# StevenWang30/R-PCC

Hardware: AMD Instinct MI355X
Metric: frames/s (64E, 64x2048 range img), projection->segmentation->model->quantise (higher is better)
Workload: dtype f32

## Files before the change

include/rpcc_hip.h:

```cpp
#ifndef RPCC_HIP_H
#define RPCC_HIP_H

#include <stddef.h>
#include <stdint.h>

#ifdef __cplusplus
extern "C" {
#endif

#define RPCC_OK 0
#define RPCC_ERR_ARG (-1)
#define RPCC_ERR_HIP (-2)
#define RPCC_MAX_CLUSTERS 254
#define RPCC_MAX_BATCH 65535
#define RPCC_INFO_INTS 8
#define RPCC_FPS_BRUTEFORCE 1
#define RPCC_FPS_FMA1 2
#define RPCC_FPS_FMA2 4
#define RPCC_FPS_TIE_CUDA 8



#define RPCC_ABI_VERSION 105
int rpcc_version(void);
// ... 18 lines not shown
int rpcc_beam_index_build(const double *angles, int H, void *out);
size_t rpcc_project_beams_scratch_bytes(int64_t total, int B, int P);
int rpcc_project_beams(const float *points, int point_stride_bytes, const int64_t *offsets, int64_t total, int B, rpcc_geom g,
                       const void *beams_dev, float *ri, void *scratch, size_t scratch_bytes, void *stream);
int rpcc_project_beams_check(const float *xyz, int64_t total, rpcc_geom g, const void *beams_dev, uint64_t *counts, void *stream);

size_t rpcc_intensity_scratch_bytes(int B, int P);
int rpcc_intensity_encode(const float *rows, const int64_t *offsets, int64_t total, int B, rpcc_geom g, const float *ri, float scale,
                          uint8_t *payload, int64_t payload_stride, int32_t *nbytes, uint8_t *image, float *owner_intensity, int32_t *orphans,
                          void *scratch, size_t scratch_bytes, void *stream);
int rpcc_intensity_decode(const uint8_t *payload, int64_t payload_stride, const int32_t *nbytes, const void *labels, int label_bytes, int B,
                          int P, float *intensity, int32_t *status, void *stream);

#define RPCC_STREAM_E_SUBPIXEL 11
size_t rpcc_subpixel_scratch_bytes(int B, int P);
int rpcc_subpixel_encode(const float *rows, const int64_t *offsets, int64_t total, int B, rpcc_geom g, const float *ri, int bits,
                         uint8_t *payload, int64_t payload_stride, int32_t *nbytes, uint8_t *codes, int32_t *orphans, void *scratch,
                         size_t scratch_bytes, void *stream);
int rpcc_subpixel_decode(const uint8_t *payload, int64_t payload_stride, const int32_t *nbytes, const void *labels, int label_bytes,
                         const float *ri_rec, const double *tables, int H, int W, int B, float *points, int32_t *status, void *stream);

int rpcc_ground_ransac(const float *ri, const float *tm, int B, int P, uint32_t seed, const int64_t *frame_ids,
                       double *ground, int32_t *inliers, void *stream);

int rpcc_ground_mask(const float *ri, const float *tm, const double *ground, double threshold, int B, int H, int W,
                     float *temp, int32_t *info, void *fps_table, void *stream);
size_t rpcc_fps_table_bytes(int B, int H, int W);

int rpcc_fps_xyz(int B, int N, int M, const float *points, float *temp, int32_t *idx, void *stream);

int rpcc_fps_range(const float *ri, const float *tm, float *temp, const int32_t *info, int B, int H, int W, int M,
                   int32_t *cen_pix, float *centers, int flags,
                   const void *fps_table , void *stream);

int rpcc_fps_xyz_bruteforce(int B, int N, int M, const float *points, float *temp, int32_t *idx, void *stream);
int rpcc_fps_xyz_mode(int B, int N, int M, const float *points, float *temp, int32_t *idx, int flags, void *stream);
int rpcc_fps_xyz_probe(int B, int N, const float *points, int32_t *marks, void *stream);

int rpcc_assign(const float *ri, const float *tm, const double *ground, const float *centers, int B, int H, int W,
                int M, uint8_t *seg, void *stream);

int rpcc_point_model(const float *ri, const uint8_t *seg, const double *ground, int B, int P, int M, float *model,
                     int32_t *counts, void *ws, void *stream);

size_t rpcc_plane_workspace_bytes(int B, int P, int M);
int rpcc_plane_model(const float *ri, const float *tm, const uint8_t *seg, const double *ground, int B, int P, int M,
// ... 164 lines not shown
```

r-pcc_amd/_lib.py:

```python
import ctypes as C
import os

import torch

_HERE = os.path.dirname(os.path.abspath(__file__))
LIB_PATH = os.environ.get("RPCC_HIP_LIB") or os.path.join(_HERE, "lib", "librpcc_hip.so")


MAX_GROUPS = 4


class Geom(C.Structure):
    _fields_ = [("H", C.c_int32), ("W", C.c_int32), ("horizontal_fov", C.c_float), ("vertical_max", C.c_float),
                ("vertical_min", C.c_float)]


class BatchIO(C.Structure):
    _fields_ = [("xyz", C.c_void_p), ("offsets", C.c_void_p), ("total", C.c_int64), ("tm", C.c_void_p),
                ("ground", C.c_void_p), ("ground_seed", C.c_int64), ("frame_ids", C.c_void_p), ("ri", C.c_void_p),
                ("seg", C.c_void_p), ("cen_pix", C.c_void_p), ("centers", C.c_void_p), ("model", C.c_void_p),
                ("counts", C.c_void_p), ("q16", C.c_void_p), ("nnz", C.c_void_p), ("info", C.c_void_p),
                ("flags", C.c_int32), ("timer", C.c_void_p), ("model_method", C.c_int32), ("plane_cos_cut", C.c_double),
                ("plane_seed", C.c_int64), ("nonuniform", C.c_void_p), ("salience", C.c_void_p), ("key_point_map", C.c_void_p),
                ("point_stride_bytes", C.c_int32)]
# ... 40 lines not shown
    pass


_VP, _I, _I64, _F, _D = C.c_void_p, C.c_int, C.c_int64, C.c_float, C.c_double
_SIGS = {
    "rpcc_version": (C.c_int, []),
    "rpcc_last_error": (C.c_char_p, []),
    "rpcc_project_scratch_bytes": (C.c_size_t, [_I64, _I, _I]),
    "rpcc_project_fastpath_check": (C.c_int, [_VP, _I64, Geom, _VP, _VP]),
    "rpcc_project": (C.c_int, [_VP, _VP, _I64, _I, Geom, _VP, _VP, C.c_size_t, _VP]),
    "rpcc_project_strided": (C.c_int, [_VP, _I, _VP, _I64, _I, Geom, _VP, _VP, C.c_size_t, _VP]),
    "rpcc_beam_index_bytes": (C.c_size_t, [_I]),
    "rpcc_beam_index_build": (C.c_int, [_VP, _I, _VP]),
    "rpcc_project_beams_scratch_bytes": (C.c_size_t, [_I64, _I, _I]),
    "rpcc_project_beams": (C.c_int, [_VP, _I, _VP, _I64, _I, Geom, _VP, _VP, _VP, C.c_size_t, _VP]),
    "rpcc_project_beams_check": (C.c_int, [_VP, _I64, Geom, _VP, _VP, _VP]),
    "rpcc_intensity_scratch_bytes": (C.c_size_t, [_I, _I]),
    "rpcc_intensity_encode": (C.c_int, [_VP, _VP, _I64, _I, Geom, _VP, _F, _VP, _I64, _VP, _VP, _VP, _VP, _VP, C.c_size_t, _VP]),
    "rpcc_intensity_decode": (C.c_int, [_VP, _I64, _VP, _VP, _I, _I, _I, _VP, _VP, _VP]),
    "rpcc_subpixel_scratch_bytes": (C.c_size_t, [_I, _I]),
    "rpcc_subpixel_encode": (C.c_int, [_VP, _VP, _I64, _I, Geom, _VP, _I, _VP, _I64, _VP, _VP, _VP, _VP, C.c_size_t, _VP]),
    "rpcc_subpixel_decode": (C.c_int, [_VP, _I64, _VP, _VP, _I, _VP, _VP, _I, _I, _I, _VP, _VP, _VP]),
    "rpcc_ground_ransac": (C.c_int, [_VP, _VP, _I, _I, C.c_uint32, _VP, _VP, _VP, _VP]),
    "rpcc_ground_mask": (C.c_int, [_VP, _VP, _VP, _D, _I, _I, _I, _VP, _VP, _VP, _VP]),
    "rpcc_fps_table_bytes": (C.c_size_t, [_I, _I, _I]),
    "rpcc_fps_xyz": (C.c_int, [_I, _I, _I, _VP, _VP, _VP, _VP]),
    "rpcc_fps_xyz_bruteforce": (C.c_int, [_I, _I, _I, _VP, _VP, _VP, _VP]),
    "rpcc_fps_xyz_mode": (C.c_int, [_I, _I, _I, _VP, _VP, _VP, _I, _VP]),
    "rpcc_fps_xyz_probe": (C.c_int, [_I, _I, _VP, _VP, _VP]),
    "rpcc_fps_range": (C.c_int, [_VP, _VP, _VP, _VP, _I, _I, _I, _I, _VP, _VP, _I, _VP, _VP]),
    "rpcc_assign": (C.c_int, [_VP, _VP, _VP, _VP, _I, _I, _I, _I, _VP, _VP]),
    "rpcc_point_model": (C.c_int, [_VP, _VP, _VP, _I, _I, _I, _VP, _VP, _VP, _VP]),
    "rpcc_predict_quantize": (C.c_int, [_VP, _VP, _VP, _VP, _VP, _VP, _F, _I, _I, _I, _VP, _VP, _VP, _VP, _VP, _VP]),
    "rpcc_intra_predict": (C.c_int, [_VP, _VP, _VP, _I, _I, _I, _VP, _VP]),
    "rpcc_assign_wide": (C.c_int, [_VP, _VP, _VP, _VP, _I, _I, _I, _I, _VP, _VP]),
    "rpcc_point_model_wide": (C.c_int, [_VP, _VP, _VP, _I, _I, _I, _VP, _VP, _VP, _VP]),
    "rpcc_predict_quantize_wide": (C.c_int, [_VP, _VP, _VP, _VP, _VP, _VP, _F, _I, _I, _I, _VP, _VP, _VP, _VP, _VP, _VP]),
    "rpcc_intra_predict_wide": (C.c_int, [_VP, _VP, _VP, _I, _I, _I, _VP, _VP]),
    "rpcc_extract_features_wide": (C.c_int, [_VP, _VP, _I, _I, _I, _I, _I, _I, _I, _I, _VP, _VP, _VP]),
    "rpcc_salience_wide": (C.c_int, [_VP, _VP, C.POINTER(C.c_int32), C.POINTER(C.c_float), _I, _I, _I, _I, _I, _VP, _VP, _VP]),
    "rpcc_plane_model_wide": (C.c_int, [_VP, _VP, _VP, _VP, _I, _I, _I, _D, C.c_uint32, _VP, _VP, _VP, _VP, _VP, _VP]),
    "rpcc_extract_features": (C.c_int, [_VP, _VP, _I, _I, _I, _I, _I, _I, _I, _I, _VP, _VP, _VP]),
    "rpcc_salience": (C.c_int, [_VP, _VP, C.POINTER(C.c_int32), C.POINTER(C.c_float), _I, _I, _I, _I, _I, _VP, _VP, _VP]),
    "rpcc_backproject": (C.c_int, [_VP, _VP, _I, _I, _VP, _VP]),
    "rpcc_codec_workspace_bytes": (C.c_size_t, [_I, _I, _I]),
    "rpcc_contour_encode": (C.c_int, [_VP, _I, _I, _I, _VP, _VP, _VP, _VP, _VP]),
# ... 112 lines not shown
```

r-pcc_amd/csrc/rpcc_hip.hip:

```cpp
#include <hip/hip_runtime.h>
#include <limits.h>
#include <math.h>
#include <stdint.h>
#include <stdio.h>
#include <string.h>

#include <algorithm>
#include <mutex>
#include <new>
#include <type_traits>
#include <utility>
#include <vector>
#include "../../include/rpcc_hip.h"
#include "rpcc_device.h"
#include "ref_rules.h"

using namespace rpcc;

static thread_local char g_err[512] = "";
static int set_err(int code, const char *fmt, const char *a = "", const char *b = "") {
    snprintf(g_err, sizeof(g_err), fmt, a, b);
    return code;
}
#define HIP_TRY(expr)                                                                      \
// ... 764 lines not shown
    __threadfence();
    __syncthreads();
    for (int p = threadIdx.x; p < P; p += FIXUP_THREADS)
        if (__hip_atomic_load(&img[p], __ATOMIC_RELAXED, __HIP_MEMORY_SCOPE_AGENT) == RI_EMPTY) img[p] = 0u;
}

static inline int band_bins_even(int P) { return (((P + BIN_PX - 1) / BIN_PX) + 1) & ~1; }
static inline int64_t pix_chunk_ids(int64_t total, int B) { return ((total > 0 ? total : 0) >> PIX_CH_SHIFT) + B; }
struct ProjectLayout { int32_t *lastz, *flags; BandBins bb; size_t atomic_bytes, bytes; };
static ProjectLayout project_layout(void *scratch, int64_t total, int B, int P) {
    const size_t nbe = (size_t)band_bins_even(P), ids = (size_t)pix_chunk_ids(total, B);
    Carve c(scratch);
    ProjectLayout l;
    l.lastz = c.take<int32_t>((size_t)B * P * 4, 4);
    l.flags = c.take<int32_t>((size_t)B * 8 * 4, 4);
    l.atomic_bytes = c.bytes(); c.take(256, 1);
    l.bb.nbe = (int)nbe;
    l.bb.ocursor = c.take<uint32_t>((size_t)B * nbe * 4, 16); l.bb.counts = c.take<uint32_t>(ids * nbe * 4, 16); l.bb.lists = c.take(ids * nbe * SHARE_BYTES, 16);
    l.bb.olists = c.take<uint2>((nbe / 2) * (size_t)((total > 0 ? total : 0) + B) * 8 + 16, 16);
    l.bytes = c.bytes();
    return l;
}
extern "C" size_t rpcc_project_scratch_bytes(int64_t total, int B, int P) { return project_layout(nullptr, total, B, P).bytes; }

extern "C" int rpcc_project_fastpath_check(const float *xyz, int64_t total, rpcc_geom g, uint64_t *counts, void *stream) {
    ARG_TRY(xyz && counts && total > 0 && g.H > 0 && g.W > 0);
    hipStream_t st = (hipStream_t)stream;
    HIP_TRY(hipMemsetAsync(counts, 0, 5 * sizeof(uint64_t), st));
    project_fastcheck_kernel<<<4096, 256, 0, st>>>(xyz, total, g, pix_fast_cfg(g), reinterpret_cast<unsigned long long *>(counts));
    LAUNCH_CHECK();
    return RPCC_OK;
}

static int launch_project(const float *xyz, const int64_t *offsets, int64_t total, int64_t base, int B, rpcc_geom g,
                          float *ri, void *scratch, size_t scratch_bytes, hipStream_t st, const float *tz_plane = nullptr,
                          int32_t *zcnt = nullptr, const BatchInit *init = nullptr, const int32_t *epoch = nullptr, int ps = 3) {
    const bool cleared = init != nullptr;
    const int P = g.H * g.W;
    uint32_t *rb = reinterpret_cast<uint32_t *>(ri);
    const ProjectLayout pl = project_layout(scratch, total, B, P);
    int32_t *lastz = pl.lastz, *flags = pl.flags;
    const dim3 fg((P + 1023) / 1024 < 64 ? (P + 1023) / 1024 : 64, B);
    const unsigned nb = (unsigned)((total + 255) / 256);
    const unsigned nb_small = nb < 2048 ? (nb ? nb : 1) : 2048;
    BandBins bb = pl.bb;
    const bool fast = scratch_bytes >= pl.bytes && bb.nbe <= PIX_MAX_BANDS && total < ((int64_t)1 << 32);
    if (fast) {
        HIP_TRY(hipMemsetAsync(bb.ocursor, 0, (size_t)B * bb.nbe * 4, st));
        if (!cleared) HIP_TRY(hipMemsetAsync(flags, 0, (size_t)(B + 1) * 4, st));
        BatchInit bi;
        memset(&bi, 0, sizeof(bi));
        if (init) bi = *init;
        if (zcnt && !cleared) HIP_TRY(hipMemsetAsync(zcnt, 0, rs_count_words(B) * 4, st));
        const unsigned pix_wgs = (unsigned)std::max<int64_t>(std::min<int64_t>(pix_chunk_ids(total, B), 256 * PIX_WG_PER_CU), 1);
        if (ps == 4) project_pix_kernel<4><<<pix_wgs, PIX_THREADS, 0, st>>>(xyz, offsets, total, base, B, g, pix_fast_cfg(g), bb, flags, epoch, bi);
        else project_pix_kernel<3><<<pix_wgs, PIX_THREADS, 0, st>>>(xyz, offsets, total, base, B, g, pix_fast_cfg(g), bb, flags, epoch, bi);
        HIP_TRY(ensure_dyn_lds(reinterpret_cast<const void *>(&project_band_kernel), BAND_PX * 4));
        const int nbands = (P + BAND_PX - 1) / BAND_PX;
        const int band_wgs = 8 * std::min(((B + 7) / 8) * nbands, std::max(BAND_WG_PER_XCD / nbands, 1) * nbands);
        project_band_kernel<<<band_wgs + (total > 0 ? B : 0), BAND_THREADS, BAND_PX * 4, st>>>(
            bb, offsets, base, B, P, rb, flags, tz_plane, -1.5f, rs_chunk_px(P), tz_plane ? zcnt : nullptr, epoch, band_wgs, xyz, g, lastz, ps);
        LAUNCH_CHECK();
        return RPCC_OK;
    }
    if (zcnt && !cleared) HIP_TRY(hipMemsetAsync(zcnt, 0, rs_count_words(B) * 4, st));
    if (init && init->on) batch_init_kernel<<<256, 256, 0, st>>>(*init);
    project_fill_kernel<false><<<fg, 256, 0, st>>>(rb, lastz, flags, P);
    LAUNCH_CHECK();
    if (total > 0) {
// ... 450 lines not shown
    return ransac_refit<RS_RU>(pts, wcnt, thr_f, plane, sred);
}

#define RS_WC_H 104
#define RS_WC_SLOT_BYTES (RS_WC_H * 4 + RS_WC_H * 20 + RS_WC_H * 32)
static_assert(RS_WC_SLOT_BYTES % 8 == 0 && (RS_WC_H * 24) % 8 == 0, "the fp64 planes of a slot are 8-byte aligned");
struct WcSlot { int32_t *cnt; float *hyp; double *hypd; };
__host__ __device__ __forceinline__ int32_t *wc_flags_of(char *wc) { return reinterpret_cast<int32_t *>(wc); }
__host__ __device__ __forceinline__ WcSlot wc_slot_of(char *wc, int nframes, int b) {
    char *p = wc + (((size_t)nframes * 4 + 63) & ~(size_t)63) + (size_t)b * RS_WC_SLOT_BYTES;
    WcSlot w;
    w.cnt = reinterpret_cast<int32_t *>(p); w.hyp = reinterpret_cast<float *>(w.cnt + RS_WC_H);
    w.hypd = reinterpret_cast<double *>(p + RS_WC_H * 24);
    return w;
}
__host__ __device__ __forceinline__ char *rs_wc_of(const int32_t *zcnt, int B, int P) {
    return reinterpret_cast<char *>((reinterpret_cast<uintptr_t>(rs_zmask_of(zcnt, B)) + (size_t)B * (size_t)(P >> 2) + 63) & ~(uintptr_t)63);
}

#define RS_CU 16
#define RS_GROUND_MAXH 104
#define RS_GROUND_PU 4
#define RS_VGPR_ATTR
__device__ __forceinline__ void ground_ransac_body(const float *__restrict__ ri_all,
                                                   const float *__restrict__ tm, int P, float zthr,
                                                   int max_pts, int min_pts, int ransac_n, int iters,
                                                   double thr, uint32_t seed0, int raw,
                                                   double *__restrict__ ground,
                                                   int32_t *__restrict__ ninl,
                                                   const int32_t *__restrict__ zcnt,
                                                   const int64_t *__restrict__ frame_ids, const int b, const int nframes,
                                                   char *__restrict__ wc = nullptr) {
    extern __shared__ __attribute__((aligned(16))) unsigned char rs_smem[];
    double *sred = reinterpret_cast<double *>(rs_smem);
    double *swin = sred + 6 * RS_NT;
    int *sbest = reinterpret_cast<int *>(swin + 64 + RS_MAX_HYP * 4);
    int *swave = sbest + 32;
    float *list = reinterpret_cast<float *>(swave + 16);
    const int tid = threadIdx.x, lane = tid & 63, wave = tid >> 6;
    const float *ri = ri_all + (int64_t)b * P;
    DBG_STAMP(0);
    constexpr int CPW = RS_CHUNKS / (RS_THREADS / 64);
    const int per_wave = CPW * ((((P + RS_CHUNKS - 1) / RS_CHUNKS) + 63) & ~63);
    const int w0 = wave * per_wave, w1 = min(P, w0 + per_wave);
    const bool have_cnt = zcnt != nullptr && zcnt[b * (RS_CHUNKS + 1) + RS_CHUNKS] != 0;
    auto zval = [&](int p) -> float {
        float r = ri[p];
        if (raw && f2u(r) == RI_EMPTY) r = 0.0f;
        return r * tm[3 * p + 2];
    };
    int cnt = 0;
    if (have_cnt)
        for (int q = 0; q < CPW; q++) cnt += zcnt[b * (RS_CHUNKS + 1) + wave * CPW + q];
    for (int p0 = w0; p0 < w1 && !have_cnt; p0 += 64 * 8) {
        float zv[8];
#pragma unroll
        for (int u = 0; u < 8; u++) zv[u] = zval(min(p0 + u * 64 + lane, P - 1));
#pragma unroll
        for (int u = 0; u < 8; u++) cnt += __popcll(__ballot(p0 + u * 64 + lane < w1 && zv[u] < zthr));
    }
    if (lane == 0) swave[wave] = cnt;
    __syncthreads();
    DBG_STAMP(1);
    int nc = 0, base = 0;
    for (int w = 0; w < RS_THREADS / 64; w++) { if (w < wave) base += swave[w]; nc += swave[w]; }
    RsPoints pts;
    pts.ri = ri; pts.tm = tm; pts.lds = nullptr; pts.n = P; pts.raw = raw;
    const bool small_prod = (unsigned long long)nc * (unsigned long long)max_pts < (1ull << 32);
    UDiv32 by_nc = {0u, 0u};
    if (nc > max_pts && small_prod) {
        by_nc = udiv32_make((uint32_t)__builtin_amdgcn_readfirstlane(nc));
        by_nc.magic = (uint32_t)__builtin_amdgcn_readfirstlane((int)by_nc.magic);
        by_nc.shift = (uint32_t)__builtin_amdgcn_readfirstlane((int)by_nc.shift);
    }
    const bool have_bytes = have_cnt && zcnt[b * (RS_CHUNKS + 1) + RS_CHUNKS] == 3 && (P & 63) == 0 && !raw;
    if (nc >= min_pts && have_bytes) {
        const uint8_t *zm = rs_zmask_of(zcnt, nframes) + (int64_t)b * (P >> 2);
        uint32_t *listp = reinterpret_cast<uint32_t *>(list);
        const bool sub = nc > max_pts;
        const uint32_t ncu = (uint32_t)nc, maxu = (uint32_t)max_pts;
        const int nwords = P >> 6;
        uint32_t run = 0u;
        __syncthreads();
        for (int wi0 = 0; wi0 < nwords; wi0 += RS_THREADS) {
            const int wi = wi0 + tid;
            const int pw = wi << 6;
            unsigned long long word = 0ull;
            if (wi < nwords) {
                const uint4 v = ld_at(reinterpret_cast<const uint4 *>(zm), (uint32_t)(pw >> 2));
                const uint32_t d[4] = {v.x, v.y, v.z, v.w};
#pragma unroll
                for (int j = 0; j < 4; j++) {
                    const uint32_t x = d[j] & 0x0F0F0F0Fu;
                    const uint32_t h = (x | (x >> 4)) & 0x00FF00FFu;
                    word |= (unsigned long long)((h | (h >> 8)) & 0xFFFFu) << (16 * j);
                }
            }
            const uint32_t c = (uint32_t)__popcll(word);
            const uint32_t incl = dpp_scan_incl_u32(c);
            if (lane == 63) swave[wave] = (int)incl;
            __syncthreads();
            uint32_t before = 0u, all = 0u;
            for (int w = 0; w < RS_THREADS / 64; w++) { const uint32_t t = (uint32_t)swave[w]; if (w < wave) before += t; all += t; }
            __syncthreads();
            uint32_t i = run + before + incl - c;
            run += all;
            if (c) {
                if (!sub) {
                    while (word) { listp[3 * i] = (uint32_t)pw + (uint32_t)__builtin_ctzll(word); i++; word &= word - 1ull; }
                } else {
                    uint32_t slot, a;
                    if (small_prod) { slot = udiv32(i * maxu, by_nc); a = i * maxu - slot * ncu; }
                    else { const unsigned long long pr = (unsigned long long)i * maxu; slot = (uint32_t)(pr / ncu); a = (uint32_t)(pr - (unsigned long long)slot * ncu); }
                    while (word) {
                        const uint32_t t = a + maxu;
                        const bool keep = t >= ncu;
                        if (keep) listp[3 * slot] = (uint32_t)pw + (uint32_t)__builtin_ctzll(word);
                        a = keep ? t - ncu : t;
                        slot += keep ? 1u : 0u;
                        word &= word - 1ull;
                    }
                }
            }
        }
        __syncthreads();
        DBG_STAMP(8);
        const int nl = sub ? max_pts : nc;
        constexpr int LU = 10;
        for (int s0 = tid; s0 < nl; s0 += RS_THREADS * LU) {
            float r[LU];
            f32x3 ray[LU];
#pragma unroll
            for (int u = 0; u < LU; u++) {
                const int sl = s0 + u * RS_THREADS;
                const uint32_t pp = listp[3 * (sl < nl ? sl : s0)];
                r[u] = ld_at(ri, pp * 4u);
                ray[u] = ld_at(reinterpret_cast<const f32x3 *>(tm), pp * 12u);
            }
#pragma unroll
            for (int u = 0; u < LU; u++) {
                const int sl = s0 + u * RS_THREADS;
                if (sl < nl) { list[3 * sl] = r[u] * ray[u].x; list[3 * sl + 1] = r[u] * ray[u].y; list[3 * sl + 2] = r[u] * ray[u].z; }
            }
        }
        pts.lds = list;
        pts.n = nl;
    } else if (nc >= min_pts) {
        int run = base;
        for (int p00 = w0; p00 < w1; p00 += 64 * RS_CU) {
            float xv[RS_CU], yv[RS_CU], zv[RS_CU];
#pragma unroll
            for (int u = 0; u < RS_CU; u++) {
                const uint32_t p = (uint32_t)min(p00 + u * 64 + lane, P - 1);
                float r = ld_at(ri, p * 4u);
                if (raw && f2u(r) == RI_EMPTY) r = 0.0f;
                const f32x3 ray = ld_at(reinterpret_cast<const f32x3 *>(tm), p * 12u);
                xv[u] = r * ray.x; yv[u] = r * ray.y; zv[u] = r * ray.z;
            }
#pragma unroll
            for (int u = 0; u < RS_CU; u++) {
                const int p = p00 + u * 64 + lane;
                const bool c = p < w1 && zv[u] < zthr;
                const unsigned long long m = __ballot(c);
                if (c) {
                    const long long i = run + __popcll(m & ((1ull << lane) - 1ull));
                    bool keep = true;
                    long long slot = i;
                    if (nc > max_pts) {
                        if (small_prod) {
                            const uint32_t a = (uint32_t)i * (uint32_t)max_pts;
                            const uint32_t sl = udiv32(a, by_nc);
                            slot = sl;
                            keep = udiv32(a + (uint32_t)max_pts, by_nc) > sl;
                        } else {
                            slot = (i * max_pts) / nc;
                            keep = ((i + 1) * max_pts) / nc > slot;
                        }
                    }
                    if (keep) { list[3 * slot] = xv[u]; list[3 * slot + 1] = yv[u]; list[3 * slot + 2] = zv[u]; }
                }
                run += __popcll(m);
            }
        }
        pts.lds = list;
        pts.n = nc > max_pts ? max_pts : nc;
    }
    __syncthreads();
    DBG_STAMP(2);
    double plane[4];
    (void)ransac_n;
    const uint32_t fid = frame_ids ? (uint32_t)frame_ids[b] : (uint32_t)b;
    const bool defer = pts.lds == nullptr && wc != nullptr && P >= 10 && iters <= RS_GROUND_MAXH;
    if (wc != nullptr && tid == 0) wc_flags_of(wc)[b] = defer ? 1 : 0;
    if (defer) {
        float *hyp = reinterpret_cast<float *>(sred);
        double *hypd = swin + 64;
        ransac_hypotheses<10>(pts, iters, seed0 + fid, hyp, hypd);
        __syncthreads();
        const WcSlot w = wc_slot_of(wc, nframes, b);
        for (int q = tid; q < RS_WC_H; q += RS_THREADS) w.cnt[q] = 0;
        for (int q = tid; q < 5 * RS_WC_H; q += RS_THREADS) w.hyp[q] = q < 5 * iters ? hyp[q] : 0.0f;
        for (int q = tid; q < 4 * iters; q += RS_THREADS) w.hypd[q] = hypd[q];
        return;
    }
    const int inl = ransac_plane_wg<10, RS_THREADS, RS_GROUND_MAXH, RS_GROUND_PU, RsPoints, false, 1>(pts, iters, thr, seed0 + fid, plane, sred, swin, sbest);
    DBG_STAMP(6);
    if (tid == 0) {
        ground[4 * b] = plane[0]; ground[4 * b + 1] = plane[1]; ground[4 * b + 2] = plane[2]; ground[4 * b + 3] = plane[3];
        if (ninl) ninl[b] = inl;
    }
}
__global__ __launch_bounds__(RS_THREADS) RS_VGPR_ATTR void ground_ransac_kernel(const float *__restrict__ ri_all,
                                                                   const float *__restrict__ tm, int P, float zthr,
                                                                   int max_pts, int min_pts, int ransac_n, int iters,
                                                                   double thr, uint32_t seed0, int raw,
                                                                   double *__restrict__ ground,
                                                                   int32_t *__restrict__ ninl,
                                                                   const int32_t *__restrict__ zcnt,
                                                                   const int64_t *__restrict__ frame_ids, char *__restrict__ wc) {
    ground_ransac_body(ri_all, tm, P, zthr, max_pts, min_pts, ransac_n, iters, thr, seed0, raw, ground, ninl, zcnt, frame_ids, blockIdx.x, gridDim.x, wc);
}
struct RansacGroupArgs {
    const float *ri_all, *tm;
    int P;
    uint32_t seed0;
    double *ground;
    const int32_t *zcnt;
    const int64_t *frame_ids;
    char *wc;
    int iters;
};
struct RansacMulti {
    int n, first[RPCC_MAX_GROUPS + 1];
    RansacGroupArgs a[RPCC_MAX_GROUPS];
};
__global__ __launch_bounds__(RS_THREADS) RS_VGPR_ATTR void ground_ransac_multi_kernel(const RansacMulti m, float zthr, int max_pts, int min_pts,
                                                                                      int ransac_n, int iters, double thr) {
    const int gi = multi_group_of(m.first, m.n, blockIdx.x);
    const RansacGroupArgs &a = m.a[gi];
    ground_ransac_body(a.ri_all, a.tm, a.P, zthr, max_pts, min_pts, ransac_n, iters, thr, a.seed0, 0, a.ground, nullptr, a.zcnt, a.frame_ids,
                       (int)blockIdx.x - m.first[gi], m.first[gi + 1] - m.first[gi], a.wc);
}

// ... 81 lines not shown
    }
    double plane[4] = {0, 0, 1, 0};
    if (wcnt >= 0) { plane[0] = w.hypd[4 * wh]; plane[1] = w.hypd[4 * wh + 1]; plane[2] = w.hypd[4 * wh + 2]; plane[3] = w.hypd[4 * wh + 3]; }
    RsPoints pts;
    pts.ri = a.ri_all + (int64_t)b * a.P; pts.tm = a.tm; pts.lds = nullptr; pts.n = a.P; pts.raw = 0;
    ransac_refit<8>(pts, wcnt, (float)thr, plane, sred);
    if (threadIdx.x == 0) { a.ground[4 * b] = plane[0]; a.ground[4 * b + 1] = plane[1]; a.ground[4 * b + 2] = plane[2]; a.ground[4 * b + 3] = plane[3]; }
}

#define RS_GROUND_MAX_PTS 5000
#define RS_GROUND_MIN_PTS 800
static inline size_t ground_ransac_lds_bytes() {
    return (size_t)6 * RS_NT * 8 + (64 + RS_MAX_HYP * 4) * 8 + 32 * 4 + 16 * 4 + (size_t)RS_GROUND_MAX_PTS * 3 * 4;
}
static int launch_ground_wc(const RansacMulti &m, hipStream_t st) {
    bool any = false;
    for (int i = 0; i < m.n; i++) any = any || m.a[i].wc != nullptr;
    if (!any) return RPCC_OK;
    ground_wc_score_kernel<<<WC_SCORE_WGS, WC_SCORE_THREADS, 0, st>>>(m, 0.1);
    ground_wc_refit_kernel<<<m.first[m.n], RS_NT, 0, st>>>(m, 0.1);
    LAUNCH_CHECK();
    return RPCC_OK;
}
static int launch_ground_ransac(const float *ri, const float *tm, int B, int P, uint32_t seed0, bool raw, double *ground,
                                int32_t *ninl, hipStream_t st, const int32_t *zcnt = nullptr,
                                const int64_t *frame_ids = nullptr) {
    const int max_pts = RS_GROUND_MAX_PTS, min_pts = RS_GROUND_MIN_PTS;
    const size_t sh = ground_ransac_lds_bytes();
    HIP_TRY(ensure_dyn_lds(reinterpret_cast<const void *>(&ground_ransac_kernel), (int)sh));
    const bool defer = zcnt != nullptr && !raw && ninl == nullptr;
    char *wc = defer ? rs_wc_of(zcnt, B, P) : nullptr;
    ground_ransac_kernel<<<B, RS_THREADS, sh, st>>>(ri, tm, P, -1.5f, max_pts, min_pts, 10, 100, 0.1, seed0, raw ? 1 : 0,
                                                    ground, ninl, zcnt, frame_ids, wc);
    LAUNCH_CHECK();
    if (defer) {
        RansacMulti m;
        m.n = 1; m.first[0] = 0; m.first[1] = B;
        m.a[0] = {ri, tm, P, seed0, ground, zcnt, frame_ids, wc, 100};
        return launch_ground_wc(m, st);
    }
    return RPCC_OK;
}
static int launch_ground_ransac_multi(const RansacMulti &m, hipStream_t st) {
    const size_t sh = ground_ransac_lds_bytes();
    HIP_TRY(ensure_dyn_lds(reinterpret_cast<const void *>(&ground_ransac_multi_kernel), (int)sh));
    ground_ransac_multi_kernel<<<m.first[m.n], RS_THREADS, sh, st>>>(m, -1.5f, RS_GROUND_MAX_PTS, RS_GROUND_MIN_PTS, 10, 100, 0.1);
    LAUNCH_CHECK();
    return launch_ground_wc(m, st);
}

extern "C" int rpcc_ground_ransac(const float *ri, const float *tm, int B, int P, uint32_t seed, const int64_t *frame_ids,
                                  double *ground, int32_t *inliers, void *stream) {
    ARG_TRY(B > 0 && B <= RPCC_MAX_BATCH && P > 0 && ri && tm && ground);
    return launch_ground_ransac(ri, tm, B, P, seed, false, ground, inliers, (hipStream_t)stream, nullptr, frame_ids);
}

// ... 845 lines not shown
    float4 *pts4 = c.take<float4>((size_t)B * P * 16);
    return {order, pts4, c.bytes()};
}
struct BatchLayout {
    WsLayout L;
    int32_t *epoch, *kpn = nullptr; char *proj_scratch, *extra = nullptr; float *temp, *rays_soa, *tiletab, *label_acc = nullptr;
    size_t proj_bytes, bytes;
};
static BatchLayout batch_layout(void *ws, int B, int P, int M, int64_t total_points, bool general) {
    Carve c(ws);
    BatchLayout l;
    l.L = ws_layout(ws, B, P, M); c.take(l.L.bytes); l.epoch = c.take<int32_t>(256);
    l.proj_bytes = round_up(project_layout(nullptr, total_points, B, P).bytes, 256); l.proj_scratch = c.take(l.proj_bytes);
    l.temp = c.take<float>((size_t)B * P * 4);
    l.rays_soa = c.take<float>((size_t)3 * P * 4 + 256, 4);
    l.tiletab = c.take<float>(0, 4);
    const size_t tab_bytes = fps_tab_bound_bytes(B, P), ksz = round_up((size_t)B * (M + 2) * 4, 256);
    Carve t(l.tiletab);
    t.take(tab_bytes + 256);
    if (general) {
        l.extra = t.take(plane_layout(nullptr, B, P).bytes);
        l.kpn = t.take<int32_t>(ksz, 4); l.label_acc = t.take<float>(ksz, 4); t.take(256, 1);
    }
    char *handoff_end = reinterpret_cast<char *>(wc_slot_of(rs_wc_of(reinterpret_cast<int32_t *>(l.tiletab), B, P), B, B).cnt);
    l.bytes = handoff_end <= reinterpret_cast<char *>(l.tiletab) + tab_bytes ? c.bytes() + t.bytes() : 0;
    return l;
}
static size_t batch_ws_bytes(int B, int P, int M, int64_t total_points, bool general) {
    const size_t n = B > 0 && P > 0 && M > 0 ? batch_layout(nullptr, B, P, M, total_points, general).bytes : 0;
    return n ? n + 4096 : 0;
}
extern "C" size_t rpcc_workspace_bytes(int B, int P, int M, int64_t total_points) { return batch_ws_bytes(B, P, M, total_points, false); }
extern "C" size_t rpcc_workspace_bytes_general(int B, int P, int M, int64_t total_points) { return batch_ws_bytes(B, P, M, total_points, true); }

#define SCAN_U 16
#define SCAN_THREADS 256
struct ScanArgs {
    const float *ri;
    const uint8_t *seg;
    const double *ground;
    int P, M, KP, T, KP2;
    const int64_t *sums;
    const int32_t *flags;
    uint32_t *hist;
    float *model;
    int32_t *counts, *nnz;
};
// ... 943 lines not shown
    int rc;
    if (t.nu && (rc = launch_nonuniform(t.ri, seg, t.B, t.H, t.W, t.M, t.nu, t.counts, t.key_point_map, t.salience, t.kpn, t.label_acc, st))) return rc;
    return launch_predict_quantize(t.ri, t.tm, seg, t.model, t.acc, t.label_acc, nullptr, t.B, t.P(), t.M, t.q16, nullptr, nullptr, t.ws, st, t.epoch);
}

enum { ST_PROJECT, ST_GROUND , ST_MASK, ST_FPS , ST_ASSIGN_LABELS, ST_PLANES , ST_QUANTISE, ST_COUNT };
template <class L>
static int run_stage(const BatchPlan &p, int stage, hipStream_t st) {
    const rpcc_batch_io *io = p.io;
    const int Bs = p.Bs, M = p.M, P = p.P;
    int rc;
    switch (stage) {
    case ST_PROJECT:
        if (p.beams) {
            batch_init_kernel<<<256, 256, 0, st>>>(p.bi);
            LAUNCH_CHECK();
            return launch_project_beams(io->xyz, io->offsets, p.npts, Bs, p.g, p.beams, io->ri, p.proj_scratch, p.proj_bytes, st,
                                        point_floats(io->point_stride_bytes));
        }
        return launch_project(io->xyz, io->offsets, p.npts, 0, Bs, p.g, io->ri, p.proj_scratch, p.proj_bytes, st,
                              p.rays_soa + 2 * (int64_t)P, p.zcnt, &p.bi, p.epoch, point_floats(io->point_stride_bytes));
    case ST_GROUND:
        if (!p.fit_ground) return RPCC_OK;
        return launch_ground_ransac(io->ri, io->tm, Bs, P, (uint32_t)io->ground_seed, false, io->ground, nullptr, st, p.zcnt, io->frame_ids);
    case ST_MASK:
        return launch_ground_mask(io->ri, io->tm, io->ground, p.ground_threshold, Bs, p.g.H, p.g.W, p.temp, io->info,
                                  p.tiled ? p.tiletab : nullptr, st, false, true);
    case ST_FPS:
        return launch_fps_range(io->ri, io->tm, p.temp, io->info, Bs, p.g.H, p.g.W, M, io->cen_pix, io->centers, io->flags, false,
                                p.tiled ? p.tiletab : nullptr, io->timer, st, p.rays_soa);
    case ST_ASSIGN_LABELS:
        if ((rc = launch_batch_assign<L>(p, st))) return rc;
        return tail_labels<L>(p.tail, st);
    case ST_PLANES:
        return tail_planes(p.tail, st);
    case ST_QUANTISE:
        return tail_quantise<L>(p.tail, st);
    }
    return RPCC_ERR_ARG;
}

static int check_batch_io(const rpcc_batch_io *io, int B, rpcc_geom g, int M, const void *ws, bool wide = false) {
    ARG_TRY(io != nullptr && ws != nullptr && B > 0 && B <= RPCC_MAX_BATCH && M > 0 && M <= (wide ? RPCC_MAX_CLUSTERS_WIDE : RPCC_MAX_CLUSTERS) &&
            g.H > 1 && g.W > 0);
    ARG_TRY(io->offsets && io->tm && io->ground && io->ri && io->seg && io->cen_pix && io->centers && io->model &&
            io->counts && io->q16 && io->nnz && io->info);
    ARG_TRY((io->flags & ~(RPCC_FPS_BRUTEFORCE | RPCC_FPS_MODE_BITS)) == 0);
// ... 424 lines not shown
```

r-pcc_amd/ops.py:

```python
import ctypes as C
import functools
import math

import numpy as np
import torch

from . import _lib
from ._lib import Geom, BatchIO, check, ptr, stream

DEFAULT_CLUSTERS = 100


def make_geom(H, W, horizontal_FOV, vertical_max, vertical_min):
    return Geom(int(H), int(W), float(horizontal_FOV), float(vertical_max), float(vertical_min))


def transform_map(H, W, horizontal_FOV, vertical_max, vertical_min, vertical_angle=None):
    vfov = vertical_max - vertical_min
    if vertical_angle is not None:
        alt = [float(a) for a in beam_table(vertical_angle, H)]
    else:
        alt = [vfov * (h / (H - 1)) + vertical_min for h in range(H)]
    azi = [horizontal_FOV * (w / W) for w in range(W)]
    ca = np.array([math.cos(a) for a in alt]); sa = np.array([math.sin(a) for a in alt])
# ... 184 lines not shown
                                          ptr(tables), H, W, B, ptr(out), ptr(status), stream()))
    return out, status


def _frame_ids(frame_ids, B, device):
    if frame_ids is None:
        return None
    if not torch.is_tensor(frame_ids):
        frame_ids = torch.as_tensor(np.asarray(frame_ids, dtype=np.int64))
    frame_ids = frame_ids.to(device=device, dtype=torch.int64).contiguous()
    assert frame_ids.numel() == B, "one identity per frame"
    return frame_ids


def ground_ransac(ri, tm, seed=0, frame_ids=None):
    B = ri.shape[0]
    P = ri[0].numel()
    ground = torch.empty((B, 4), dtype=torch.float64, device=_dev(ri))
    inl = torch.empty((B,), dtype=torch.int32, device=_dev(ri))
    fid = _frame_ids(frame_ids, B, _dev(ri))
    check(_lib.lib().rpcc_ground_ransac(ptr(ri), ptr(tm), B, P, int(seed) & 0xFFFFFFFF, ptr(fid), ptr(ground), ptr(inl),
                                        stream()))
    return ground, inl


def ground_mask(ri, tm, ground, threshold, fps_table=False, table=None):
    B, H, W = ri.shape
    P = H * W
    temp = torch.empty((B, P), dtype=torch.float32, device=_dev(ri))
    info = torch.empty((B, _lib.INFO_INTS), dtype=torch.int32, device=_dev(ri))
    tab = None
    if fps_table:
        tab = torch.empty(_lib.lib().rpcc_fps_table_bytes(B, H, W) // 4, dtype=torch.float32, device=_dev(ri)) if table is None else table
    check(_lib.lib().rpcc_ground_mask(ptr(ri), ptr(tm), ptr(ground), float(threshold), B, H, W, ptr(temp), ptr(info),
                                      ptr(tab), stream()))
    return (temp, info, tab) if fps_table else (temp, info)


def fps_xyz(points, npoint, temp=None, bruteforce=False, fma=0, cuda_tie=False):
    B, N, _ = points.shape
    if temp is None:
        temp = torch.full((B, N), 1e10, dtype=torch.float32, device=_dev(points))
    idx = torch.empty((B, npoint), dtype=torch.int32, device=_dev(points))
    mode = _lib.fps_mode_flags(fma, cuda_tie)
    if mode:
        check(_lib.lib().rpcc_fps_xyz_mode(B, N, npoint, ptr(points), ptr(temp), ptr(idx), mode, stream()))
# ... 455 lines not shown
```

Before: 382,000.

## Split ground RANSAC candidate gathering into a chunk-parallel pre-kernel

```diff
diff --git a/include/rpcc_hip.h b/include/rpcc_hip.h
--- a/include/rpcc_hip.h
+++ b/include/rpcc_hip.h
@@ -64,6 +64,7 @@
 
 int rpcc_ground_ransac(const float *ri, const float *tm, int B, int P, uint32_t seed, const int64_t *frame_ids,
                        double *ground, int32_t *inliers, void *stream);
+int rpcc_ground_candidates(const float *ri, const float *tm, int B, int P, const int32_t *handoff, float *cand, void *stream);
 
 int rpcc_ground_mask(const float *ri, const float *tm, const double *ground, double threshold, int B, int H, int W,
                      float *temp, int32_t *info, void *fps_table, void *stream);
diff --git a/r-pcc_amd/_lib.py b/r-pcc_amd/_lib.py
--- a/r-pcc_amd/_lib.py
+++ b/r-pcc_amd/_lib.py
@@ -86,6 +86,7 @@
     "rpcc_subpixel_encode": (C.c_int, [_VP, _VP, _I64, _I, Geom, _VP, _I, _VP, _I64, _VP, _VP, _VP, _VP, C.c_size_t, _VP]),
     "rpcc_subpixel_decode": (C.c_int, [_VP, _I64, _VP, _VP, _I, _VP, _VP, _I, _I, _I, _VP, _VP, _VP]),
     "rpcc_ground_ransac": (C.c_int, [_VP, _VP, _I, _I, C.c_uint32, _VP, _VP, _VP, _VP]),
+    "rpcc_ground_candidates": (C.c_int, [_VP, _VP, _I, _I, _VP, _VP, _VP]),
     "rpcc_ground_mask": (C.c_int, [_VP, _VP, _VP, _D, _I, _I, _I, _VP, _VP, _VP, _VP]),
     "rpcc_fps_table_bytes": (C.c_size_t, [_I, _I, _I]),
     "rpcc_fps_xyz": (C.c_int, [_I, _I, _I, _VP, _VP, _VP, _VP]),
diff --git a/r-pcc_amd/csrc/rpcc_hip.hip b/r-pcc_amd/csrc/rpcc_hip.hip
--- a/r-pcc_amd/csrc/rpcc_hip.hip
+++ b/r-pcc_amd/csrc/rpcc_hip.hip
@@ -810,6 +810,9 @@
     return l;
 }
 extern "C" size_t rpcc_project_scratch_bytes(int64_t total, int B, int P) { return project_layout(nullptr, total, B, P).bytes; }
+static inline bool project_binned(const ProjectLayout &pl, int64_t total, size_t scratch_bytes) {
+    return scratch_bytes >= pl.bytes && pl.bb.nbe <= PIX_MAX_BANDS && total < ((int64_t)1 << 32);
+}
 
 extern "C" int rpcc_project_fastpath_check(const float *xyz, int64_t total, rpcc_geom g, uint64_t *counts, void *stream) {
     ARG_TRY(xyz && counts && total > 0 && g.H > 0 && g.W > 0);
@@ -832,7 +835,7 @@
     const unsigned nb = (unsigned)((total + 255) / 256);
     const unsigned nb_small = nb < 2048 ? (nb ? nb : 1) : 2048;
     BandBins bb = pl.bb;
-    const bool fast = scratch_bytes >= pl.bytes && bb.nbe <= PIX_MAX_BANDS && total < ((int64_t)1 << 32);
+    const bool fast = project_binned(pl, total, scratch_bytes);
     if (fast) {
         HIP_TRY(hipMemsetAsync(bb.ocursor, 0, (size_t)B * bb.nbe * 4, st));
         if (!cleared) HIP_TRY(hipMemsetAsync(flags, 0, (size_t)(B + 1) * 4, st));
@@ -1329,6 +1332,102 @@
 #define RS_GROUND_MAXH 104
 #define RS_GROUND_PU 4
 #define RS_VGPR_ATTR
+__device__ __forceinline__ unsigned long long rs_unpack_word(const uint4 v) {
+    const uint32_t d[4] = {v.x, v.y, v.z, v.w};
+    unsigned long long word = 0ull;
+#pragma unroll
+    for (int j = 0; j < 4; j++) {
+        const uint32_t x = d[j] & 0x0F0F0F0Fu;
+        const uint32_t h = (x | (x >> 4)) & 0x00FF00FFu;
+        word |= (unsigned long long)((h | (h >> 8)) & 0xFFFFu) << (16 * j);
+    }
+    return word;
+}
+__device__ __forceinline__ void rs_slot_of(uint32_t i, uint32_t maxu, uint32_t ncu, bool small_prod, const UDiv32 by_nc, uint32_t &slot, uint32_t &a) {
+    if (small_prod) { slot = udiv32(i * maxu, by_nc); a = i * maxu - slot * ncu; }
+    else { const unsigned long long pr = (unsigned long long)i * maxu; slot = (uint32_t)(pr / ncu); a = (uint32_t)(pr - (unsigned long long)slot * ncu); }
+}
+__host__ __device__ __forceinline__ float *rs_cand_of(const int32_t *zcnt, int B, int P) {
+    return reinterpret_cast<float *>((reinterpret_cast<uintptr_t>(wc_slot_of(rs_wc_of(zcnt, B, P), B, B).cnt) + 255) & ~(uintptr_t)255);
+}
+
+#define GC_THREADS 128
+#define GC_U 4
+__global__ __launch_bounds__(GC_THREADS) void ground_candidates_kernel(const float *__restrict__ ri_all, const float *__restrict__ tm, int P,
+                                                                       int rs_chunk, int max_pts, int min_pts,
+                                                                       const int32_t *__restrict__ zcnt, float *__restrict__ cand) {
+    __shared__ uint32_t swave[2][GC_THREADS / 64];
+    const int ch = blockIdx.x, b = blockIdx.y, nframes = gridDim.y;
+    const int tid = threadIdx.x, lane = tid & 63, wave = tid >> 6;
+    const int32_t *zc = zcnt + b * (RS_CHUNKS + 1);
+    if (zc[RS_CHUNKS] != 3 || (P & 63) != 0) return;
+    int nc = 0, first = 0;
+    for (int q = 0; q < RS_CHUNKS; q++) { const int t = zc[q]; if (q < ch) first += t; nc += t; }
+    if (nc < min_pts || zc[ch] == 0) return;
+    const bool sub = nc > max_pts;
+    const uint32_t ncu = (uint32_t)nc, maxu = (uint32_t)max_pts, nl = sub ? maxu : ncu;
+    const bool small_prod = (unsigned long long)nc * (unsigned long long)max_pts < (1ull << 32);
+    UDiv32 by_nc = {0u, 0u};
+    if (sub && small_prod) {
+        by_nc = udiv32_make((uint32_t)__builtin_amdgcn_readfirstlane(nc));
+        by_nc.magic = (uint32_t)__builtin_amdgcn_readfirstlane((int)by_nc.magic);
+        by_nc.shift = (uint32_t)__builtin_amdgcn_readfirstlane((int)by_nc.shift);
+    }
+    const uint8_t *zm = rs_zmask_of(zcnt, nframes) + (int64_t)b * (P >> 2);
+    const float *ri = ri_all + (int64_t)b * P;
+    f32x3 *out = reinterpret_cast<f32x3 *>(cand + (int64_t)b * max_pts * 3);
+    const int cwords = rs_chunk >> 6, w_beg = ch * cwords, w_end = min(P >> 6, w_beg + cwords);
+    uint32_t run = (uint32_t)first;
+    int par = 0;
+    for (int wi0 = w_beg; wi0 < w_end; wi0 += GC_THREADS, par ^= 1) {
+        const int wi = wi0 + tid;
+        const uint32_t pw = (uint32_t)wi << 6;
+        unsigned long long word = 0ull;
+        if (wi < w_end) word = rs_unpack_word(ld_at(reinterpret_cast<const uint4 *>(zm), pw >> 2));
+        const uint32_t c = (uint32_t)__popcll(word);
+        const uint32_t incl = dpp_scan_incl_u32(c);
+        if (lane == 63) swave[par][wave] = incl;
+        __syncthreads();
+        uint32_t before = 0u, all = 0u;
+        for (int w = 0; w < GC_THREADS / 64; w++) { const uint32_t t = swave[par][w]; if (w < wave) before += t; all += t; }
+        const uint32_t i = run + before + incl - c;
+        run += all;
+        unsigned long long kept = word;
+        uint32_t slot = i;
+        if (sub && c) {
+            uint32_t a;
+            rs_slot_of(i, maxu, ncu, small_prod, by_nc, slot, a);
+            kept = 0ull;
+            for (unsigned long long w = word; w; w &= w - 1ull) {
+                const uint32_t t = a + maxu;
+                const bool keep = t >= ncu;
+                if (keep) kept |= w & (0ull - w);
+                a = keep ? t - ncu : t;
+            }
+        }
+        while (kept) {
+            uint32_t pp[GC_U];
+            bool on[GC_U];
+            float r[GC_U];
+            f32x3 ray[GC_U];
+#pragma unroll
+            for (int u = 0; u < GC_U; u++) {
+                on[u] = kept != 0ull;
+                pp[u] = pw + (on[u] ? (uint32_t)__builtin_ctzll(kept) : 0u);
+                kept &= kept - 1ull;
+                r[u] = ld_at(ri, pp[u] * 4u);
+                ray[u] = ld_at(reinterpret_cast<const f32x3 *>(tm), pp[u] * 12u);
+            }
+#pragma unroll
+            for (int u = 0; u < GC_U; u++) {
+                if (on[u] && slot + u < nl) st_at(out, (slot + u) * 12u, f32x3{r[u] * ray[u].x, r[u] * ray[u].y, r[u] * ray[u].z});
+            }
+            slot += GC_U;
+        }
+    }
+}
+
+template <bool LIST = false>
 __device__ __forceinline__ void ground_ransac_body(const float *__restrict__ ri_all,
                                                    const float *__restrict__ tm, int P, float zthr,
                                                    int max_pts, int min_pts, int ransac_n, int iters,
@@ -1337,7 +1436,7 @@
                                                    int32_t *__restrict__ ninl,
                                                    const int32_t *__restrict__ zcnt,
                                                    const int64_t *__restrict__ frame_ids, const int b, const int nframes,
-                                                   char *__restrict__ wc = nullptr) {
+                                                   char *__restrict__ wc = nullptr, const float *__restrict__ cand = nullptr) {
     extern __shared__ __attribute__((aligned(16))) unsigned char rs_smem[];
     double *sred = reinterpret_cast<double *>(rs_smem);
     double *swin = sred + 6 * RS_NT;
@@ -1347,6 +1446,31 @@
     const int tid = threadIdx.x, lane = tid & 63, wave = tid >> 6;
     const float *ri = ri_all + (int64_t)b * P;
     DBG_STAMP(0);
+    RsPoints pts;
+    pts.ri = ri; pts.tm = tm; pts.lds = nullptr; pts.n = P; pts.raw = raw;
+    bool handed = false;
+    if constexpr (LIST) handed = zcnt[b * (RS_CHUNKS + 1) + RS_CHUNKS] == 3 && (P & 63) == 0 && !raw;
+    if (handed) {
+        int nc = 0;
+        for (int q = 0; q < RS_CHUNKS; q++) nc += zcnt[b * (RS_CHUNKS + 1) + q];
+        if (nc >= min_pts) {
+            static_assert((6 * RS_NT * 8 + (64 + RS_MAX_HYP * 4) * 8 + 32 * 4 + 16 * 4) % 16 == 0, "the LDS list is 16-byte aligned");
+            const int nl = nc > max_pts ? max_pts : nc, n16 = (3 * nl) >> 2;
+            const float *src = cand + (int64_t)b * max_pts * 3;
+            constexpr int RS_LU = 8;
+            for (int q0 = tid; q0 - tid < n16; q0 += RS_THREADS * RS_LU) {
+                uint4 v[RS_LU];
+#pragma unroll
+                for (int u = 0; u < RS_LU; u++) v[u] = ld_at(reinterpret_cast<const uint4 *>(src), (uint32_t)min(q0 + u * RS_THREADS, n16 - 1) * 16u);
+#pragma unroll
+                for (int u = 0; u < RS_LU; u++)
+                    if (q0 + u * RS_THREADS < n16) reinterpret_cast<uint4 *>(list)[q0 + u * RS_THREADS] = v[u];
+            }
+            if (4 * n16 + tid < 3 * nl) list[4 * n16 + tid] = src[4 * n16 + tid];
+            pts.lds = list;
+            pts.n = nl;
+        }
+    } else {
     constexpr int CPW = RS_CHUNKS / (RS_THREADS / 64);
     const int per_wave = CPW * ((((P + RS_CHUNKS - 1) / RS_CHUNKS) + 63) & ~63);
     const int w0 = wave * per_wave, w1 = min(P, w0 + per_wave);
@@ -1371,8 +1495,6 @@
     DBG_STAMP(1);
     int nc = 0, base = 0;
     for (int w = 0; w < RS_THREADS / 64; w++) { if (w < wave) base += swave[w]; nc += swave[w]; }
-    RsPoints pts;
-    pts.ri = ri; pts.tm = tm; pts.lds = nullptr; pts.n = P; pts.raw = raw;
     const bool small_prod = (unsigned long long)nc * (unsigned long long)max_pts < (1ull << 32);
     UDiv32 by_nc = {0u, 0u};
     if (nc > max_pts && small_prod) {
@@ -1380,7 +1502,7 @@
         by_nc.magic = (uint32_t)__builtin_amdgcn_readfirstlane((int)by_nc.magic);
         by_nc.shift = (uint32_t)__builtin_amdgcn_readfirstlane((int)by_nc.shift);
     }
-    const bool have_bytes = have_cnt && zcnt[b * (RS_CHUNKS + 1) + RS_CHUNKS] == 3 && (P & 63) == 0 && !raw;
+    const bool have_bytes = !LIST && have_cnt && zcnt[b * (RS_CHUNKS + 1) + RS_CHUNKS] == 3 && (P & 63) == 0 && !raw;
     if (nc >= min_pts && have_bytes) {
         const uint8_t *zm = rs_zmask_of(zcnt, nframes) + (int64_t)b * (P >> 2);
         uint32_t *listp = reinterpret_cast<uint32_t *>(list);
@@ -1393,16 +1515,7 @@
             const int wi = wi0 + tid;
             const int pw = wi << 6;
             unsigned long long word = 0ull;
-            if (wi < nwords) {
-                const uint4 v = ld_at(reinterpret_cast<const uint4 *>(zm), (uint32_t)(pw >> 2));
-                const uint32_t d[4] = {v.x, v.y, v.z, v.w};
-#pragma unroll
-                for (int j = 0; j < 4; j++) {
-                    const uint32_t x = d[j] & 0x0F0F0F0Fu;
-                    const uint32_t h = (x | (x >> 4)) & 0x00FF00FFu;
-                    word |= (unsigned long long)((h | (h >> 8)) & 0xFFFFu) << (16 * j);
-                }
-            }
+            if (wi < nwords) word = rs_unpack_word(ld_at(reinterpret_cast<const uint4 *>(zm), (uint32_t)(pw >> 2)));
             const uint32_t c = (uint32_t)__popcll(word);
             const uint32_t incl = dpp_scan_incl_u32(c);
             if (lane == 63) swave[wave] = (int)incl;
@@ -1417,8 +1530,7 @@
                     while (word) { listp[3 * i] = (uint32_t)pw + (uint32_t)__builtin_ctzll(word); i++; word &= word - 1ull; }
                 } else {
                     uint32_t slot, a;
-                    if (small_prod) { slot = udiv32(i * maxu, by_nc); a = i * maxu - slot * ncu; }
-                    else { const unsigned long long pr = (unsigned long long)i * maxu; slot = (uint32_t)(pr / ncu); a = (uint32_t)(pr - (unsigned long long)slot * ncu); }
+                    rs_slot_of(i, maxu, ncu, small_prod, by_nc, slot, a);
                     while (word) {
                         const uint32_t t = a + maxu;
                         const bool keep = t >= ncu;
@@ -1454,10 +1566,11 @@
         pts.n = nl;
     } else if (nc >= min_pts) {
         int run = base;
-        for (int p00 = w0; p00 < w1; p00 += 64 * RS_CU) {
-            float xv[RS_CU], yv[RS_CU], zv[RS_CU];
-#pragma unroll
-            for (int u = 0; u < RS_CU; u++) {
+        constexpr int CU = LIST ? 4 : RS_CU;
+        for (int p00 = w0; p00 < w1; p00 += 64 * CU) {
+            float xv[CU], yv[CU], zv[CU];
+#pragma unroll
+            for (int u = 0; u < CU; u++) {
                 const uint32_t p = (uint32_t)min(p00 + u * 64 + lane, P - 1);
                 float r = ld_at(ri, p * 4u);
                 if (raw && f2u(r) == RI_EMPTY) r = 0.0f;
@@ -1465,7 +1578,7 @@
                 xv[u] = r * ray.x; yv[u] = r * ray.y; zv[u] = r * ray.z;
             }
 #pragma unroll
-            for (int u = 0; u < RS_CU; u++) {
+            for (int u = 0; u < CU; u++) {
                 const int p = p00 + u * 64 + lane;
                 const bool c = p < w1 && zv[u] < zthr;
                 const unsigned long long m = __ballot(c);
@@ -1492,6 +1605,7 @@
         pts.lds = list;
         pts.n = nc > max_pts ? max_pts : nc;
     }
+    }
     __syncthreads();
     DBG_STAMP(2);
     double plane[4];
@@ -1517,6 +1631,7 @@
         if (ninl) ninl[b] = inl;
     }
 }
+template <bool LIST>
 __global__ __launch_bounds__(RS_THREADS) RS_VGPR_ATTR void ground_ransac_kernel(const float *__restrict__ ri_all,
                                                                    const float *__restrict__ tm, int P, float zthr,
                                                                    int max_pts, int min_pts, int ransac_n, int iters,
@@ -1524,8 +1639,10 @@
                                                                    double *__restrict__ ground,
                                                                    int32_t *__restrict__ ninl,
                                                                    const int32_t *__restrict__ zcnt,
-                                                                   const int64_t *__restrict__ frame_ids, char *__restrict__ wc) {
-    ground_ransac_body(ri_all, tm, P, zthr, max_pts, min_pts, ransac_n, iters, thr, seed0, raw, ground, ninl, zcnt, frame_ids, blockIdx.x, gridDim.x, wc);
+                                                                   const int64_t *__restrict__ frame_ids, char *__restrict__ wc,
+                                                                   const float *__restrict__ cand) {
+    ground_ransac_body<LIST>(ri_all, tm, P, zthr, max_pts, min_pts, ransac_n, iters, thr, seed0, raw, ground, ninl, zcnt, frame_ids, blockIdx.x, gridDim.x,
+                             wc, cand);
 }
 struct RansacGroupArgs {
     const float *ri_all, *tm;
@@ -1653,16 +1770,34 @@
     LAUNCH_CHECK();
     return RPCC_OK;
 }
+static void launch_ground_candidates(const float *ri, const float *tm, int B, int P, const int32_t *zcnt, float *cand, hipStream_t st) {
+    ground_candidates_kernel<<<dim3(RS_CHUNKS, B), GC_THREADS, 0, st>>>(ri, tm, P, rs_chunk_px(P), RS_GROUND_MAX_PTS, RS_GROUND_MIN_PTS, zcnt, cand);
+}
+extern "C" int rpcc_ground_candidates(const float *ri, const float *tm, int B, int P, const int32_t *handoff, float *cand, void *stream) {
+    ARG_TRY(B > 0 && B <= RPCC_MAX_BATCH && P > 0 && ri && tm && handoff && cand);
+    ARG_TRY((reinterpret_cast<uintptr_t>(handoff) & 15u) == 0 && (reinterpret_cast<uintptr_t>(cand) & 15u) == 0);
+    launch_ground_candidates(ri, tm, B, P, handoff, cand, (hipStream_t)stream);
+    LAUNCH_CHECK();
+    return RPCC_OK;
+}
 static int launch_ground_ransac(const float *ri, const float *tm, int B, int P, uint32_t seed0, bool raw, double *ground,
                                 int32_t *ninl, hipStream_t st, const int32_t *zcnt = nullptr,
-                                const int64_t *frame_ids = nullptr) {
+                                const int64_t *frame_ids = nullptr, bool handed = false) {
     const int max_pts = RS_GROUND_MAX_PTS, min_pts = RS_GROUND_MIN_PTS;
+    static_assert(RS_GROUND_MAX_PTS % 4 == 0, "a frame's candidate list starts at a multiple of 16 bytes");
     const size_t sh = ground_ransac_lds_bytes();
-    HIP_TRY(ensure_dyn_lds(reinterpret_cast<const void *>(&ground_ransac_kernel), (int)sh));
     const bool defer = zcnt != nullptr && !raw && ninl == nullptr;
     char *wc = defer ? rs_wc_of(zcnt, B, P) : nullptr;
-    ground_ransac_kernel<<<B, RS_THREADS, sh, st>>>(ri, tm, P, -1.5f, max_pts, min_pts, 10, 100, 0.1, seed0, raw ? 1 : 0,
-                                                    ground, ninl, zcnt, frame_ids, wc);
+    if (handed && zcnt != nullptr && !raw) {
+        float *cand = rs_cand_of(zcnt, B, P);
+        HIP_TRY(ensure_dyn_lds(reinterpret_cast<const void *>(&ground_ransac_kernel<true>), (int)sh));
+        launch_ground_candidates(ri, tm, B, P, zcnt, cand, st);
+        ground_ransac_kernel<true><<<B, RS_THREADS, sh, st>>>(ri, tm, P, -1.5f, max_pts, min_pts, 10, 100, 0.1, seed0, 0, ground, ninl, zcnt, frame_ids, wc, cand);
+    } else {
+        HIP_TRY(ensure_dyn_lds(reinterpret_cast<const void *>(&ground_ransac_kernel<false>), (int)sh));
+        ground_ransac_kernel<false><<<B, RS_THREADS, sh, st>>>(ri, tm, P, -1.5f, max_pts, min_pts, 10, 100, 0.1, seed0, raw ? 1 : 0,
+                                                               ground, ninl, zcnt, frame_ids, wc, nullptr);
+    }
     LAUNCH_CHECK();
     if (defer) {
         RansacMulti m;
@@ -2554,7 +2689,7 @@
         l.extra = t.take(plane_layout(nullptr, B, P).bytes);
         l.kpn = t.take<int32_t>(ksz, 4); l.label_acc = t.take<float>(ksz, 4); t.take(256, 1);
     }
-    char *handoff_end = reinterpret_cast<char *>(wc_slot_of(rs_wc_of(reinterpret_cast<int32_t *>(l.tiletab), B, P), B, B).cnt);
+    char *handoff_end = reinterpret_cast<char *>(rs_cand_of(reinterpret_cast<int32_t *>(l.tiletab), B, P) + (size_t)B * RS_GROUND_MAX_PTS * 3);
     l.bytes = handoff_end <= reinterpret_cast<char *>(l.tiletab) + tab_bytes ? c.bytes() + t.bytes() : 0;
     return l;
 }
@@ -3544,7 +3679,8 @@
                               p.rays_soa + 2 * (int64_t)P, p.zcnt, &p.bi, p.epoch, point_floats(io->point_stride_bytes));
     case ST_GROUND:
         if (!p.fit_ground) return RPCC_OK;
-        return launch_ground_ransac(io->ri, io->tm, Bs, P, (uint32_t)io->ground_seed, false, io->ground, nullptr, st, p.zcnt, io->frame_ids);
+        return launch_ground_ransac(io->ri, io->tm, Bs, P, (uint32_t)io->ground_seed, false, io->ground, nullptr, st, p.zcnt, io->frame_ids,
+                                    p.beams == nullptr && (P & 63) == 0 && project_binned(project_layout(nullptr, p.npts, Bs, P), p.npts, p.proj_bytes));
     case ST_MASK:
         return launch_ground_mask(io->ri, io->tm, io->ground, p.ground_threshold, Bs, p.g.H, p.g.W, p.temp, io->info,
                                   p.tiled ? p.tiletab : nullptr, st, false, true);
diff --git a/r-pcc_amd/ops.py b/r-pcc_amd/ops.py
--- a/r-pcc_amd/ops.py
+++ b/r-pcc_amd/ops.py
@@ -230,6 +230,29 @@
     check(_lib.lib().rpcc_ground_ransac(ptr(ri), ptr(tm), B, P, int(seed) & 0xFFFFFFFF, ptr(fid), ptr(ground), ptr(inl),
                                         stream()))
     return ground, inl
+
+
+GROUND_MAX_PTS, GROUND_MIN_PTS, GROUND_CHUNKS = 5000, 800, 16
+
+
+def ground_handoff(counts, valid, zbytes):
+    B = counts.shape[0]
+    words = torch.cat([counts.to(torch.int32), valid.to(torch.int32).reshape(B, 1)], dim=1).contiguous()
+    head = (B * (GROUND_CHUNKS + 1) * 4 + 15) & ~15
+    block = torch.zeros((head + zbytes.numel(),), dtype=torch.uint8, device=_dev(counts))
+    block[:B * (GROUND_CHUNKS + 1) * 4] = words.reshape(-1).view(torch.uint8)
+    block[head:] = zbytes.reshape(-1)
+    return block
+
+
+def ground_candidates(ri, tm, handoff, cand=None):
+    B = ri.shape[0]
+    P = ri[0].numel()
+    if cand is None:
+        cand = torch.full((B, GROUND_MAX_PTS, 3), float("nan"), dtype=torch.float32, device=_dev(ri))
+    assert cand.dtype == torch.float32 and cand.numel() == B * GROUND_MAX_PTS * 3
+    check(_lib.lib().rpcc_ground_candidates(ptr(ri), ptr(tm), B, P, ptr(handoff), ptr(cand), stream()))
+    return cand
 
 
 def ground_mask(ri, tm, ground, threshold, fps_table=False, table=None):
```

After: 367,500. 3.8% lower.
